# guangkun0818/speech2text

Hardware: AMD Instinct MI355X
Metric: audio-seconds/sec (train step, zipformer pruned-RNN-T) (higher is better)
Workload: dtype f32; 1 GPU; C3 zipformer pruned-RNN-T train step: chunk_size -1, 500 BPE, prune_range 5 (fbank+fwd+bwd+allreduce+ScaledAdam); accumulate_grad_batches=1, gemm_arith=bf16x2/3, per_gpu_batch=64, global_batch=64, labels_per_utt=50, parallelism=dp1

## Files before the change

### include/s2t_mi355.h

```cpp
#ifndef S2T_MI355_H_
#define S2T_MI355_H_

#ifdef __cplusplus
extern "C" {
#endif

int s2t_fbank_f32(const float* pcm, long pcm_stride, const long* num_samples, int batch,
                  const float* window400, const float* twiddle512, const int* mel_off,
                  const int* mel_k0, const float* mel_w, int nnz, int num_mel, float eps,
                  float scale_in, const float* cmvn_mean, const float* cmvn_istd, float* out,
                  int max_frames, long* out_frames, void* stream);

#define S2T_CTC_MAX_LABELS 1023
long s2t_ctc_workspace_floats(int B, int T, int Umax);
int s2t_ctc_loss_fwd_bwd(const float* logits, const long* targets, long tgt_stride,
                         const long* in_len, const long* tgt_len, int B, int T, int V, int Umax,
                         int blank, int zero_infinity, const float* grad_scale, float* workspace,
                         float* loss_per_utt, float* grad_logits, void* stream);

int s2t_fill_f32(float* p, long n, float v, void* stream);
int s2t_rnnt_row_exp(const float* x, long rows, int C, float* probs, float* rowmax, void* stream);
int s2t_rnnt_simple_pxpy(const float* am, const float* lm, const float* am_max,
                         const float* lm_max, const float* nrm, const long* symbols,
                         const long* boundary, int B, int S, int T, int C, int blank, float* px,
                         float* py, void* stream);
int s2t_rnnt_simple_w(const float* dpx, const float* dpy, const float* nrm, const float* gscale,
                      int B, int S, int T, float* W, void* stream);
int s2t_rnnt_simple_bwd(const float* am_probs, const float* lm_probs, const float* G_am,
                        const float* G_lm, const float* dpx, const float* dpy,
                        const float* gscale, const long* symbols, int B, int S, int T, int C,
                        int blank, float* d_am, float* d_lm, int accumulate, void* stream);
int s2t_mutual_info_fwd(const float* px, const float* py, const long* boundary, int B, int S,
                        int T, float* p, float* ans, void* stream);
int s2t_mutual_info_bwd(const float* px, const float* py, const long* boundary, const float* p,
                        const float* ans_grad, int B, int S, int T, float* px_grad,
                        float* py_grad, void* stream);
int s2t_rnnt_prune_ranges(const float* px_grad, const float* py_grad, const long* boundary, int B,
                          int S, int T, int s_range, long* ranges, void* stream);
int s2t_rnnt_pruned_fwd(const float* am, const float* lm, const long* ranges,
                        const long* symbols, const long* boundary, int B, int S, int T, int C,
                        int R, int blank, int act, float* px, float* py, float* lse, void* stream);
int s2t_rnnt_pruned_bwd(const float* am, const float* lm, const long* ranges,
                        const long* symbols, const float* lse, const float* dpx, const float* dpy,
                        const float* gscale, int B, int S, int T, int C, int R, int blank, int act,
                        float* d_am, float* d_lm, int accumulate, void* stream);
int s2t_rnnt_lattice_fwd(const float* logits, const long* ranges, const long* symbols,
                         const long* boundary, int B, int S, int T, int V, int R, int blank,
                         float* px, float* py, float* lse, void* stream);
int s2t_rnnt_lattice_bwd(const float* logits, const long* ranges, const long* symbols,
                         const float* lse, const float* dpx, const float* dpy,
                         const float* gscale, int B, int S, int T, int V, int R, int blank,
                         float* d_logits, void* stream);


int s2t_swoosh_fwd(const float* x, float* y, long n, float offset, float constant, void* stream);
int s2t_swoosh_bwd(const float* x, const float* g, float* d, long n, float offset, void* stream);
int s2t_biasnorm_fwd(const float* x, const float* bias, const float* log_scale, long rows, int D,
                     float* y, float* scales, void* stream);
int s2t_biasnorm_fwd_tb(const float* x, const float* bias, const float* log_scale, int T, int B, int D,
                        float* y, float* scales, void* stream);
int s2t_biasnorm_bwd_tb(const float* x, const float* bias, const float* scales, const float* g, int T,
                        int B, int D, float* dx, float* dbias, float* dls, void* stream);
int s2t_norm_bypass_fwd(const float* x, const float* bias, const float* log_scale, const float* orig,
                        const float* bypass_scale, const float* fm, int B, long rows, int D, float* out,
                        float* scales, void* stream);
int s2t_norm_bypass_bwd(const float* x, const float* bias, const float* scales, const float* orig,
                        const float* bypass_scale, const float* g, const float* fm, int B, long rows, int D,
                        float* dx, float* d_orig, float* d_bypass_scale, float* dbias, float* dls,
                        void* stream);
int s2t_biasnorm_bwd(const float* x, const float* bias, const float* scales, const float* g,
                     long rows, int D, float* dx, float* dbias, float* dls, void* stream);
long s2t_balancer_bwd_workspace_floats(void);
int s2t_balancer_bwd(const float* x, long ldx, const float* g, long ldg, long rows, int C,
                     float min_mean, float max_mean, float min_rms, float max_rms,
                     float grad_scale, float* out, long ldo, float* workspace, int parity,
                     float act_off, void* stream);
int s2t_balancer_stats(const float* x, long ldx, long rows, int C, float* stats, void* stream);
int s2t_balancer_apply(const float* x, long ldx, const float* g, long ldg, long rows, int C,
                       float min_mean, float max_mean, float min_rms, float max_rms,
                       float grad_scale, float* out, long ldo, const float* stats, float act_off,
                       void* stream);


int s2t_zipconv_fwd(const float* u, long ld, int gate_off, const unsigned char* mask, int T, int B,
                    int C, int K, int chunk, const float* wc, const float* bc, const float* wk,
                    const float* bk, const float* scale, float* y, void* stream);
int s2t_zipconv_fwd_act(const float* u, long ld, int gate_off, const unsigned char* mask, int T, int B,
                        int C, int K, int chunk, const float* wc, const float* bc, const float* wk,
                        const float* bk, const float* scale, float* y, float* y_act, int act_kind,
                        void* stream);
int s2t_zipconv_bwd(const float* u, long ld, int gate_off, const unsigned char* mask, int T, int B,
                    int C, int K, int chunk, const float* wc, const float* wk, const float* bk,
                    const float* scale, const float* dy, float* du, float* dwc, float* dbc,
                    float* dwk, float* dbk, float* dscale, float* workspace, void* stream);
int s2t_zipconv_bwd_data(const float* u, long ld, int gate_off, const unsigned char* mask, int T,
                         int B, int C, int K, int chunk, const float* wc, const float* wk,
                         const float* bk, const float* scale, const float* dy, float* du,
                         void* stream);
int s2t_zipconv_bwd_params(const float* u, long ld, int gate_off, const unsigned char* mask, int T,
                           int B, int C, int K, int chunk, const float* wc, const float* wk,
                           const float* bk, const float* scale, const float* dy, float* dwc,
                           float* dbc, float* dwk, float* dbk, float* dscale, float* workspace,
                           void* stream);
long s2t_zipconv_bwd_workspace_floats(int T, int B, int C, int K);


int s2t_relpos_attn_fwd(const float* qkp, const float* pos, const unsigned char* kpm,
                        const unsigned char* amask, int T, int B, int H, int qd, int pd, float* W,
                        void* stream);
int s2t_relpos_attn_fwd_flag(const float* qkp, const float* pos, const unsigned char* kpm,
                             const unsigned char* amask, int T, int B, int H, int qd, int pd,
                             float* W, float pen_limit, float* pen_flag, void* stream);
int s2t_relpos_attn_bwd(const float* qkp, const float* pos, const unsigned char* kpm,
                        const unsigned char* amask, int T, int B, int H, int qd, int pd,
                        const float* W, const float* dW, const float* dW0, const float* dO1,
                        const float* V1, int dv1, const float* dO2, const float* V2, int dv2,
                        int delta_given, float* delta_ws, float* dqkp, float* dpos,
                        float* workspace, void* stream);
long s2t_relpos_attn_bwd_workspace_floats(int T, int B, int H, int pd);
int s2t_attn_apply(const float* W, const float* v, int T, int B, int H, int dv, int transpose,
                   float* out, void* stream);


long s2t_linear_wgrad_workspace_floats(int R, int N, int M);
int s2t_linear_wgrad(const float* g, long ldg, const float* a, long lda, int R, int N, int M,
                     float* dW, float* db, int accumulate, float* workspace, void* stream);

int s2t_whiten_metric(float* xtx, float* colsum, long n, int G, int cg, float* cov, float* mean,
                      float* scal, float* host_metric, float* workspace, void* stream);
int s2t_whiten_prep(const float* cov, const float* mean, const float* scal, int G, int cg, float* dcov,
                    float* bias, float* sums64, void* stream);
int s2t_gemm_x3p_sq(const float* A, long lda, const unsigned short* Bp, int N, int K, float* C, long ldc,
                    int M, const float* bias, const float* other, long ld_other, float* sums, int tile,
                    void* stream);
int s2t_sumsq64(const float* g, long numel, float* sums64, void* stream);
int s2t_whiten_combine64(const float* g, const float* pg, long numel, float grad_scale,
                         const float* sums64, float* out, void* stream);
int s2t_whiten_dcov(const float* cov, const float* mean, const float* scal, int G, int cg,
                    float* dcov, float* bias, float* sums, void* stream);
int s2t_whiten_apply(const float* g, const float* pg, long numel, float grad_scale, float* sums,
                     float* out, void* stream);
int s2t_limit_param_grad(const float* x, const float* g, float lo, float hi, long n, float* out,
                         void* stream);

int s2t_bestrq_labels(const float* feats, int B, int T, int F, const float* proj, int D,
                      const float* codebooks, int ncb, int K, int T2, long* labels, void* stream);


int s2t_col2im3x3_nhwc(const float* dc, int B, int H, int W, int C, int Ho, int Wo, int sh, int sw,
                       float* dx, void* stream);

int s2t_conv3x3_c1(int mode, const float* x, const float* w, const float* bias, const float* g, int B,
                   int H, int W, int pw, int CO, float* y, float* dw, float* db, float* dx,
                   void* stream);

int s2t_conv3x3_s2(int mode, const float* x, const float* w, const float* bias, const float* g, int B,
                   int H, int W, int CI, int CO, float* y, float* dx, void* stream);

int s2t_conv3x3_gemm(int mode, const float* x, int B, int H, int W, int C, int sh, int sw, int CO,
                     const float* w2_or_g, const float* bias, float* out, float* db, void* stream);

int s2t_dwconv2d_nhwc_fwd(const float* x, const float* wgt, const float* bias, int N, int H, int W,
                          int C, int KH, int KW, int flip, float* y, void* stream);
int s2t_dwconv2d_nhwc_fwd_add(const float* x, const float* wgt, const float* bias, const float* add,
                              int N, int H, int W, int C, int KH, int KW, int flip, float* y,
                              void* stream);
long s2t_dwconv2d_wgrad_workspace_floats(int N, int H, int C, int KH, int KW);
int s2t_dwconv2d_nhwc_wgrad(const float* x, const float* dy, int N, int H, int W, int C, int KH,
                            int KW, float* workspace, float* dw, float* db, void* stream);

int s2t_optim_chunk_elems(void);
int s2t_optim_segc_floats(void);
int s2t_seg_stats(const float* p, const float* g, const int* chunk_off, const int* chunk_len,
                  int nchunks, float* partial, void* stream);
int s2t_scaled_adam_coef(const float* partial, const int* seg_chunk_begin, const int* seg_len,
                         int nchunks_all, int seg_lo, int seg_hi, float lr, float beta1,
                         float beta2, float eps, float scalar_lr_scale, float param_min_rms,
                         float param_max_rms, float scalar_max, float clip_val,
                         float clipping_scale, int step, int size_update_period,
                         int clipping_update_period, float bc2, float bc2_size, float beta2c,
                         float* param_rms, float* scale_exp_avg_sq, float* scale_grads,
                         float* model_norms, float* fstate, int* istate, float* segstat,
                         float* segc, const float* skip, void* stream);
int s2t_scaled_adam_apply(float* p, float* g, float* delta, float* exp_avg_sq,
                          const int* chunk_off, const int* chunk_len, const int* chunk_seg,
                          int nchunks, const float* segc, int zero_grad, void* stream);

int s2t_gemm_f32(int mode, const float* A, long lda, const float* B, long ldb, float* C, long ldc,
                 int M, int N, int K, const float* bias, const float* resid, long ldr,
                 const float* act_src, long lds, int act_kind, int pro_a, int pro_b, float* colsum,
                 int accumulate, void* stream);

int s2t_gemm_f32_batched(int mode, const float* A, long lda, long sA, const float* B, long ldb, long sB,
                         float* C, long ldc, long sC, int M, int N, int K, int batch, void* stream);

int s2t_gemm_f32_sq(int mode, const float* A, long lda, const float* B, long ldb, float* C, long ldc,
                    int M, int N, int K, const float* bias, const float* other, long ld_other,
                    float* sums, void* stream);
int s2t_whiten_combine(const float* g, const float* pg, long numel, float grad_scale, const float* sums,
                       float* out, void* stream);

int s2t_gemm_f32_tiled(int mode, const float* A, long lda, const float* B, long ldb, float* C,
                       long ldc, int M, int N, int K, const float* bias, const float* resid,
                       long ldr, int tile, void* stream);

int s2t_tn_x3(int set);
int s2t_tn_w(int set);
int s2t_nn_x3(int set);

int s2t_gemm_xtx(const float* x, long ldx, int R, int C, int cg, float* xtx, long ldc,
                 float* colsum, void* stream);

typedef struct S2tTnProblem {
  const float* A;
  long lda;
  const float* B;
  long ldb;
  float* C;
  long ldc;
  int M, N, K;
  float* colsum;
  float alpha;
} S2tTnProblem;
int s2t_gemm_tn_grouped(int n, const S2tTnProblem* probs, void* stream);

int s2t_smoothed_nll_fwd(const float* logits, const long* labels, long rows, int K, float scale,
                         float t_other, float t_label, float c0, float* row_loss, float* lse,
                         void* stream);
int s2t_smoothed_nll_bwd(const float* logits, const long* labels, const float* lse,
                         const float* row_weight, long rows, int K, float scale, float t_other,
                         float t_label, float* grad, void* stream);

int s2t_ctc_greedy(const float* logits, const long* lengths, int B, int T, int V, int blank,
                   long* tokens, long* out_len, void* stream);
int s2t_rnnt_greedy_stateless(const float* am, const long* lengths, const float* emb,
                              const float* conv_w, const float* lin_w, const float* lin_b,
                              const float* pre_w, const float* pre_b, int B, int T, int V, int E,
                              int D, int ctx, int act, int max_token_step, int max_out, int blank,
                              long* tokens, long* out_len, void* stream);

long s2t_rnnt_beam_workspace_bytes(int B, int T, int V, int beam_size);
int s2t_rnnt_beam_stateless(const float* am, const long* lengths, const float* emb,
                            const float* conv_w, const float* lin_w, const float* lin_b,
                            const float* pre_w, const float* pre_b, int B, int T, int V, int E,
                            int D, int ctx, int act, int blank, int beam_size, int cutoff_top_k,
                            void* workspace, long* tokens, long* frames, long* out_len,
                            float* score, void* stream);

long s2t_rnnt_stream_state_bytes(int B, int V, int ctx, int beam_size, int max_tokens);
int s2t_rnnt_stream_reset(void* state, const int* rows, int B, int V, int ctx, int beam_size,
                          int max_tokens, int blank, void* stream);
int s2t_rnnt_greedy_stateless_chunk(const float* am, const long* chunk_len, const float* emb,
                                    const float* conv_w, const float* lin_w, const float* lin_b,
                                    const float* pre_w, const float* pre_b, int B, int Tc, int V,
                                    int E, int D, int ctx, int act, int max_token_step,
                                    int max_tokens, int blank, void* state, long* tokens,
                                    long* out_len, int* overflow, void* stream);
int s2t_rnnt_beam_stateless_chunk(const float* am, const long* chunk_len, const float* emb,
                                  const float* conv_w, const float* lin_w, const float* lin_b,
                                  const float* pre_w, const float* pre_b, int B, int Tc, int V, int E,
                                  int D, int ctx, int act, int blank, int beam_size,
                                  int cutoff_top_k, int max_tokens, void* state, long* tokens,
                                  long* frames, long* out_len, float* score, long* stable_len,
                                  int* overflow, void* stream);

#define S2T_RNNT_LSTM_MAX_HIDDEN 1024
#define S2T_RNNT_LSTM_MAX_LAYERS 8
#define S2T_RNNT_LSTM_MAX_VOCAB 8192
#define S2T_RNNT_LSTM_MAX_BEAM 16
typedef struct S2tLstmLayer {
  const float* x2g_w;
  const float* x2g_b;
  const float* p2g_w;
  const float *g_gamma, *g_beta;
  const float *c_gamma, *c_beta;
} S2tLstmLayer;
typedef struct S2tRnntLstmDesc {
  int V, E, H, D, inner, num_layers, layer_norm, act;
  float in_eps, lstm_eps, out_eps;
  int pad_;
  const float* emb;
  const float *in_gamma, *in_beta;
  S2tLstmLayer layers[S2T_RNNT_LSTM_MAX_LAYERS];
  const float *lin_w, *lin_b;
  const float *out_gamma, *out_beta;
  const float *pre_w, *pre_b;
  const float *out1_w, *out1_b;
  const float *out2_w, *out2_b;
} S2tRnntLstmDesc;
long s2t_rnnt_lstm_workspace_bytes(const S2tRnntLstmDesc* desc, int B, int T, int beam_size);
int s2t_lstm_pred_step(const S2tRnntLstmDesc* desc, int R, const int* tokens, const int* emit,
                       const int* parent, const float* h_in, const float* c_in, const float* lm_in,
                       float* h_out, float* c_out, float* lm_out, void* workspace, void* stream);
int s2t_rnnt_greedy_lstm(const S2tRnntLstmDesc* desc, const float* am, const long* lengths, int B,
                         int T, int max_token_step, void* workspace, long* tokens, long* out_len,
                         void* stream);
int s2t_rnnt_beam_lstm(const S2tRnntLstmDesc* desc, const float* am, const long* lengths, int B,
                       int T, int beam_size, int cutoff_top_k, void* workspace, long* tokens,
                       long* frames, long* out_len, float* score, void* stream);

int s2t_row_energy(const float* x, long stride, const long* len, int B, int D, int mode, float* out,
                   void* stream);
int s2t_mix(const float* src, long sstride, const long* slen, const float* noise, long nstride,
// ... 313 lines not shown
```

### speech2text_amd/zip_kernels.py

```python
import ctypes
import os

import torch
import torch.nn.functional as F

from . import _native as N
from . import flat
from . import planes

_SW = {True: (4.0, 0.035), False: (1.0, 0.313261687)}


def _dev(*ts):
    for t in ts:
        if t is not None and not t.is_cuda:
            raise RuntimeError("speech2text_amd zipformer kernels run on the GPU only "
                               "(no CPU fallback); got a CPU tensor")


def _c16(t):
    t = t.contiguous()
    if t.data_ptr() % 16:
        t = t.clone()
    return t
# ... 1525 lines not shown
        w2m = w2 if w2.dim() == 2 else w2.reshape(w2.shape[0], -1)
        g2 = _rows(g)
        grads2 = (None, None)
        if not wgrad_into(w2p, b2p, g2, a):
            dw, db = linear_wgrad(g2, a, b2p is not None)
            grads2 = (dw.view(w2.shape), db)
        if ctx.bal_cfg is not None:
            dh = lt_matmul(1, g2, w2m, act_src=h, act_kind="swoosh_l", bal=ctx.bal_cfg)
        else:
            dh = lt_matmul(1, g2, w2m, act_src=h, act_kind="swoosh_l")
        grads1 = (None, None)
        if not wgrad_into(w1p, b1p, dh, x2):
            dw, db = linear_wgrad(dh, x2, b1p is not None)
            grads1 = (dw.view(w1.shape), db)
        dx = lt_matmul(1, dh, w1m).view(ctx.xshape) if ctx.needs_input_grad[0] else None
        return dx, grads1[0], grads1[1], grads2[0], grads2[1], (g if ctx.has_res else None), None


def ffn_block(x, w1, b1, w2, b2, residual=None, balancer_cfg=None):
    if not x.is_cuda:
        raise RuntimeError("speech2text_amd.ffn_block needs device tensors (HIP path only)")
    return _FfnBlock.apply(x, w1, b1, w2, b2, residual, balancer_cfg)


class _LinearColPerm(torch.autograd.Function):

    @staticmethod
    def forward(ctx, x, weight, bias, f, c):
        wp = weight.detach().view(-1, c, f).permute(0, 2, 1).reshape(-1, f * c)
        x2 = _rows(x)
        y = lt_matmul(0, x2, wp, bias)
        ctx.save_for_backward(x2, wp)
        ctx.params = (weight, bias)
        ctx.cfg = (x.shape, f, c)
        return y.view(x.shape[:-1] + (wp.shape[0],))

    @staticmethod
    def backward(ctx, g):
        x2, wp = ctx.saved_tensors
        weight, bias = ctx.params
        xshape, f, c = ctx.cfg
        g2 = _rows(g)
        dx = lt_matmul(1, g2, wp).view(xshape) if ctx.needs_input_grad[0] else None

        def compute():
            dwp, db = linear_wgrad(g2, x2, bias is not None)
            return [dwp.view(-1, f, c).permute(0, 2, 1).reshape(weight.shape), db]
        dw, db = side_param_grads((weight, bias), compute, keep=(g2, x2))
        return dx, dw, db, None, None


def linear_col_perm(x, weight, bias, f, c):
    if not x.is_cuda:
        raise RuntimeError("speech2text_amd.linear_col_perm needs device tensors (HIP path only)")
    return _LinearColPerm.apply(x, weight, bias, f, c)


def linear_pass(x, weight, bias=None):
    return _LinearPass.apply(x, weight, bias)


def linear(x, weight, bias=None, residual=None):
    if not x.is_cuda:
        raise RuntimeError("speech2text_amd.linear needs device tensors (HIP path only)")
    return _Linear.apply(x, weight, bias, residual)


def _wgrad_splitk(a, g, chunk=16384):
    R = a.shape[0]
    S = R // chunk
    if S < 4:
        return a.t().mm(g)
    main = torch.bmm(a[:S * chunk].view(S, chunk, -1).transpose(1, 2),
                     g[:S * chunk].view(S, chunk, -1)).sum(dim=0)
    if S * chunk < R:
        main = main + a[S * chunk:].t().mm(g[S * chunk:])
    return main


def linear_big_m(x, weight, bias):
    return _Linear.apply(x, weight, bias, None)


def _conv3x3_wgrad_implicit(x, g, sh, sw, has_bias):
    B, H, W, C = x.shape
    Cout = g.shape[-1]
    dw2 = torch.zeros((Cout, 9 * C), dtype=torch.float32, device=x.device)
    db = torch.zeros((Cout,), dtype=torch.float32, device=x.device) if has_bias else None
    R = g.numel() // Cout
    N.PROF[0] and N.profile_note("s2t_conv3x3_gemm", 4.0 * (x.numel() + g.numel()), 2.0 * R * Cout * 9 * C)
    N.check(N.lib().s2t_conv3x3_gemm(2, N.fp(x), B, H, W, C, sh, sw, Cout, N.fp(g), None, N.fp(dw2),
                                     N.fp(db), N.stream()), "s2t_conv3x3_gemm(wgrad)")
    return dw2.view(Cout, 3, 3, C).permute(0, 3, 1, 2), db


def _implicit_ok(x, Cout, sh=1, sw=1):
    B, H, W, C = x.shape
    rows = B * ((H - 3) // sh + 1) * ((W - 3) // sw + 1)
    return x.is_cuda and C % 4 == 0 and Cout % 4 == 0 and x.numel() < (1 << 31) and rows >= 4


class _Conv3x3Nhwc(torch.autograd.Function):

    @staticmethod
    def forward(ctx, x, weight, bias, sh, sw):
        _dev(x, weight)
        x = x.contiguous().float()
        B, H, W, C = x.shape
        Cout = weight.shape[0]
        Ho, Wo = (H - 3) // sh + 1, (W - 3) // sw + 1
        w2 = weight.permute(0, 2, 3, 1).reshape(Cout, 9 * C)
        ctx.implicit = _implicit_ok(x, Cout, sh, sw)
        pp = None
        if ctx.implicit and C % 16 == 0 and Cout % 16 == 0:
            pp = planes.adhoc_pieces(w2.detach().contiguous(), 0)
        if pp is not None:
            y = torch.empty((B * Ho * Wo, Cout), dtype=torch.float32, device=x.device)
            amap = RowMap(Ho * Wo, Wo, H * W * C, sh * W * C, sw * C, 0)
            N.check(_x3p_map(x, amap, 3 * C, [0, W * C, 2 * W * C], pp, Cout, y, Cout, None, 0, B * Ho * Wo,
                             None if bias is None else bias.detach()), "s2t_gemm_x3p_map(fwd)")
            ctx.save_for_backward(x, weight)
        elif ctx.implicit:
            y = torch.empty((B * Ho * Wo, Cout), dtype=torch.float32, device=x.device)
            N.PROF[0] and N.profile_note("s2t_conv3x3_gemm", 4.0 * (x.numel() + y.numel()),
                           2.0 * y.numel() * 9 * C)
            N.check(N.lib().s2t_conv3x3_gemm(0, N.fp(x), B, H, W, C, sh, sw, Cout, N.fp(w2),
                                             N.fp(bias), N.fp(y), None, N.stream()),
                    "s2t_conv3x3_gemm")
            ctx.save_for_backward(x, weight)
        else:
            s = x.stride()
            cols = x.as_strided((B, Ho, Wo, 3, 3 * C), (s[0], s[1] * sh, s[2] * sw, s[1], 1)) \
                .reshape(B * Ho * Wo, 9 * C)
            y = lt_matmul(0, cols, w2, bias)
            ctx.save_for_backward(cols, weight)
        ctx.cfg = (B, H, W, C, Ho, Wo, sh, sw, bias is not None)
        ctx.params = (weight, bias)
        return y.view(B, Ho, Wo, Cout)

    @staticmethod
    def backward(ctx, dy):
        xc, weight = ctx.saved_tensors
        B, H, W, C, Ho, Wo, sh, sw, has_bias = ctx.cfg
        Cout = weight.shape[0]
        g = dy.reshape(B * Ho * Wo, Cout)
        g = g if g.is_contiguous() else g.contiguous()
        if ctx.implicit:
            dweight, db = side_param_grads(
                ctx.params, lambda: list(_conv3x3_wgrad_implicit(xc, g, sh, sw, has_bias)), keep=(xc, g))
        else:
            dwmat, db = linear_wgrad(g, xc, has_bias)
            dweight = dwmat.view(Cout, 3, 3, C).permute(0, 3, 1, 2)
        dx = None
        if ctx.needs_input_grad[0] and ctx.implicit and (sh, sw) == (1, 2) and Cout % 16 == 0 \
                and C >= 16 and g.numel() * 5 < (1 << 31):
            dx = _conv3x3_s12_dgrad_map(g.view(B, Ho, Wo, Cout), weight.detach(), H, W)
        elif ctx.needs_input_grad[0] and ctx.implicit and 9 * C * Cout >= (1 << 18):
            gy = g.view(B, Ho, Wo, Cout).permute(0, 3, 1, 2)
            xin = xc.permute(0, 3, 1, 2)
            wcl = weight.contiguous(memory_format=torch.channels_last)
            dxn = torch.ops.aten.convolution_backward(gy, xin, wcl, None, [sh, sw], [0, 0], [1, 1],
                                                      False, [0, 0], 1, [True, False, False])[0]
            dx = dxn.permute(0, 2, 3, 1)
        elif ctx.needs_input_grad[0]:
            w2 = weight.permute(0, 2, 3, 1).reshape(Cout, 9 * C)
            dc = lt_matmul(1, g, w2)
            dx = torch.empty((B, H, W, C), dtype=torch.float32, device=dy.device)
            N.PROF[0] and N.profile_note("s2t_col2im3x3_nhwc", 4.0 * (dc.numel() + dx.numel()))
            N.check(N.lib().s2t_col2im3x3_nhwc(N.fp(dc), B, H, W, C, Ho, Wo, sh, sw, N.fp(dx),
                                               N.stream()), "s2t_col2im3x3_nhwc")
        return dx, dweight, db, None, None


_CONV_MAP_DGRAD_TILE = 221


_PAD_BUF = {}


def _conv3x3_s12_dgrad_map(g, wd, H, W):
    B, Ho, Wo, Cout = g.shape
    C = wd.shape[1]
    key = (B, Ho, Wo, Cout, g.device.index)
    gp = _PAD_BUF.get(key)
    if gp is None:
        _PAD_BUF.clear()
        gp = _PAD_BUF[key] = torch.zeros((B, Ho + 4, Wo + 2, Cout), dtype=torch.float32, device=g.device)
    gp[:, 2:Ho + 2, 1:Wo + 1].copy_(g)
    Wp = Wo + 2
    dx = torch.empty((B, H, W, C), dtype=torch.float32, device=g.device)
    for pw in (0, 1):
        kws = (2, 0) if pw == 0 else (1,)
        bc = torch.cat([wd[:, :, kh, kw].t() for kh in (0, 1, 2) for kw in kws], dim=1).contiguous()
        pp = planes.adhoc_pieces(bc, 0)
        if pp is None:
            raise RuntimeError("conv3x3 (map, stride 1x2): class weight outside the piece kernel's rules")
        Wc = (W - pw + 1) // 2
        amap = RowMap(H * Wc, Wc, (Ho + 4) * Wp * Cout, Wp * Cout, Cout, (2 * Wp + 1) * Cout)
        segoff = [(-kh * Wp - (1 if pw == 0 else 0)) * Cout for kh in (0, 1, 2)]
        cmap = RowMap(H * Wc, Wc, H * W * C, W * C, 2 * C, pw * C)
        N.check(_x3p_map(gp, amap, len(kws) * Cout, segoff, pp, C, dx, C, cmap, dx.numel(), B * H * Wc, None,
                         tile=_CONV_MAP_DGRAD_TILE), "s2t_gemm_x3p_map(dgrad 1x2)")
    return dx


RowMap = N.struct("S2tRowMap")


_CONV_MAP_TILE = 22


def _x3p_map(a, amap, seg, segoff, pp, ncols, out, ldc, cmap, c_elems, M, bias, tile=None):
    tile = _CONV_MAP_TILE if tile is None else tile
    if tile >= 200 and (seg % 32 or N.lib().s2t_gemm_arith() != 2):
        tile -= 200
    so = (ctypes.c_long * len(segoff))(*segoff)
    N.PROF[0] and N.profile_note("s2t_gemm_x3p_map", 4.0 * (a.numel() + out.numel()) + 6.0 * ncols * seg * len(segoff),
                                 2.0 * M * ncols * seg * len(segoff))
    return N.lib().s2t_gemm_x3p_map(_vp(a), ctypes.byref(amap), seg, len(segoff), so, ctypes.c_void_p(pp), ncols,
                                    _vp(out), ldc, None if cmap is None else ctypes.byref(cmap), c_elems, M,
                                    _vp(bias), tile, N.stream())


class _Conv3x3S2Map(torch.autograd.Function):

    @staticmethod
    def forward(ctx, x, weight, bias):
        _dev(x, weight)
        x = x.contiguous().float()
        B, H, W, C = x.shape
        Cout = weight.shape[0]
        Ho, Wo = (H - 3) // 2 + 1, (W - 3) // 2 + 1
        w2 = weight.detach().permute(0, 2, 3, 1).reshape(Cout, 9 * C).contiguous()
        pp = planes.adhoc_pieces(w2, 0)
        if pp is None:
            raise RuntimeError("conv3x3 (map): weight shape outside the piece kernel's rules")
        M = B * Ho * Wo
        y = torch.empty((M, Cout), dtype=torch.float32, device=x.device)
        amap = RowMap(Ho * Wo, Wo, H * W * C, 2 * W * C, 2 * C, 0)
        N.check(_x3p_map(x, amap, 3 * C, [0, W * C, 2 * W * C], pp, Cout, y, Cout, None, 0, M,
                         None if bias is None else bias.detach()), "s2t_gemm_x3p_map(fwd)")
        ctx.save_for_backward(x, weight)
        ctx.params = (weight, bias)
        ctx.dims = (B, H, W, C, Ho, Wo, Cout)
        return y.view(B, Ho, Wo, Cout)

    @staticmethod
    def backward(ctx, dy):
        x, weight = ctx.saved_tensors
        B, H, W, C, Ho, Wo, Cout = ctx.dims
        g = dy.contiguous().float()
        has_bias = ctx.params[1] is not None
        dweight, db = side_param_grads(
            ctx.params, lambda: list(_conv3x3_wgrad_implicit(x, g.view(-1, Cout), 2, 2, has_bias)), keep=(x, g))
        dx = None
        if ctx.needs_input_grad[0]:
            gp = F.pad(g, (0, 0, 1, 1, 1, 1))
            dx = torch.empty((B, H, W, C), dtype=torch.float32, device=g.device)
            wd = weight.detach()
            P2 = Wo + 2
            for ph in (0, 1):
                for pw in (0, 1):
                    taps = [(kh, kw) for kh in ((0, 2) if ph == 0 else (1,)) for kw in ((0, 2) if pw == 0 else (1,))]
                    bc = torch.cat([wd[:, :, kh, kw].t() for kh, kw in taps], dim=1).contiguous()
                    pp = planes.adhoc_pieces(bc, 0)
                    if pp is None:
                        raise RuntimeError("conv3x3 (map): class weight outside the piece kernel's rules")
                    Hc, Wc = (H - ph + 1) // 2, (W - pw + 1) // 2
                    amap = RowMap(Hc * Wc, Wc, (Ho + 2) * P2 * Cout, P2 * Cout, Cout, (P2 + 1) * Cout)
                    segoff = [((-1 if kh == 2 else 0) * P2 + (-1 if kw == 2 else 0)) * Cout for kh, kw in taps]
                    cmap = RowMap(Hc * Wc, Wc, H * W * C, 2 * W * C, 2 * C, (ph * W + pw) * C)
                    N.check(_x3p_map(gp, amap, Cout, segoff, pp, C, dx, C, cmap, dx.numel(), B * Hc * Wc, None),
                            "s2t_gemm_x3p_map(dgrad)")
        return dx, dweight, db


def conv3x3_s2_map_ok(x, weight, stride):
    return (x.is_cuda and tuple(stride) == (2, 2) and x.shape[-1] % 16 == 0 and weight.shape[0] % 16 == 0
            and x.shape[1] >= 3 and x.shape[2] >= 3 and x.numel() < (1 << 29) and weight.shape[1] == x.shape[-1])


def conv3x3_s2_map(x, weight, bias):
    return _Conv3x3S2Map.apply(x, weight, bias)


class _Conv3x3C1(torch.autograd.Function):

    @staticmethod
    def forward(ctx, x, weight, bias, pw, grad_scale=None):
        _dev(x, weight)
        ctx.grad_scale = grad_scale
        x3 = x.reshape(x.shape[0], x.shape[1], x.shape[2]).contiguous().float()
        B, H, W = x3.shape
        CO = weight.shape[0]
        y = torch.empty((B, H - 2, W + 2 * pw - 2, CO), dtype=torch.float32, device=x.device)
        w = weight.contiguous().float()
        N.PROF[0] and N.profile_note("s2t_conv3x3_c1", 4.0 * (x3.numel() + y.numel()))
        N.check(N.lib().s2t_conv3x3_c1(0, N.fp(x3), N.fp(w), N.fp(bias), None, B, H, W, pw, CO,
                                       N.fp(y), None, None, None, N.stream()), "s2t_conv3x3_c1")
        ctx.save_for_backward(x3, w)
        ctx.cfg = (pw, bias is not None, x.shape)
        return y

    @staticmethod
    def backward(ctx, g):
        x3, w = ctx.saved_tensors
        pw, has_bias, xshape = ctx.cfg
        B, H, W = x3.shape
        CO = w.shape[0]
        g = g.contiguous().float()
        acc = torch.zeros(CO * 10, dtype=torch.float32, device=g.device)
        L = N.lib()
        N.PROF[0] and N.profile_note("s2t_conv3x3_c1", 4.0 * (x3.numel() + g.numel()))
        N.check(L.s2t_conv3x3_c1(1, N.fp(x3), None, None, N.fp(g), B, H, W, pw, CO, None, N.fp(acc),
                                 ctypes_off(acc, CO * 9), None, N.stream()), "s2t_conv3x3_c1(wgrad)")
        dx = None
        if ctx.needs_input_grad[0]:
            dx = torch.empty_like(x3)
            N.PROF[0] and N.profile_note("s2t_conv3x3_c1", 4.0 * (g.numel() + dx.numel()))
            N.check(L.s2t_conv3x3_c1(2, None, N.fp(w), None, N.fp(g), B, H, W, pw, CO, None, None,
                                     None, N.fp(dx), N.stream()), "s2t_conv3x3_c1(dgrad)")
            dx = dx.view(xshape)
        if ctx.grad_scale is not None:
            acc = acc * float(ctx.grad_scale)
# ... 153 lines not shown
```

Before: 18070 audio-seconds/sec.

## Add direct MFMA kernel for stride-(1,2) conv3x3 input gradient

Adds a dedicated HIP kernel for the input gradient of the stride-(1,2) 3x3 conv in the subsampling frontend. It stages a padded tile of dy in LDS, pre-splits the weights into bf16 hi/lo fragments, and applies only the taps that touch each output column parity using 3-pass bf16 MFMA. This replaces the padded-copy map path and avoids materialising intermediate buffers. It only runs when Cin is 32, Cout is at most 128, and the gemm arithmetic mode is bf16x3; otherwise it falls back to the old paths. Exchanges a precision mode fixed to bf16x3 for fewer memory passes.

```diff
diff --git a/include/s2t_mi355.h b/include/s2t_mi355.h
--- a/include/s2t_mi355.h
+++ b/include/s2t_mi355.h
@@ -149,6 +149,10 @@
 
 int s2t_col2im3x3_nhwc(const float* dc, int B, int H, int W, int C, int Ho, int Wo, int sh, int sw,
                        float* dx, void* stream);
+
+long s2t_conv3x3_s12_dgrad_work_bytes(int Cin, int Cout);
+int s2t_conv3x3_s12_dgrad(const float* dy, const float* weight, int B, int H, int W, int Cin, int Cout,
+                          float* dx, void* work, void* stream);
 
 int s2t_conv3x3_c1(int mode, const float* x, const float* w, const float* bias, const float* g, int B,
                    int H, int W, int pw, int CO, float* y, float* dw, float* db, float* dx,
diff --git a/speech2text_amd/csrc/conv_dgrad.hip b/speech2text_amd/csrc/conv_dgrad.hip
--- /dev/null
+++ b/speech2text_amd/csrc/conv_dgrad.hip
@@ -0,0 +1,243 @@
+#include "common.h"
+#include "conv_dgrad_index.h"
+#include "../../include/s2t_mi355.h"
+
+namespace {
+
+typedef float f32x16 __attribute__((ext_vector_type(16)));
+typedef float f32x2 __attribute__((ext_vector_type(2)));
+typedef float f32x4 __attribute__((ext_vector_type(4)));
+typedef unsigned u32x4 __attribute__((ext_vector_type(4)));
+typedef __bf16 bf16x2 __attribute__((ext_vector_type(2)));
+typedef __bf16 bf16x8 __attribute__((ext_vector_type(8)));
+typedef const __attribute__((address_space(1))) f32x4* gf32x4p;
+typedef const __attribute__((address_space(1))) u32x4* gu32x4p;
+
+__device__ __forceinline__ void split_pair2(float x0, float x1, unsigned& p0, unsigned& p1) {
+  f32x2 x = {x0, x1};
+  p0 = __builtin_bit_cast(unsigned, __builtin_convertvector(x, bf16x2));
+  f32x2 h = {__uint_as_float(p0 << 16), __uint_as_float(p0 & 0xFFFF0000u)};
+  x = x - h;
+  p1 = __builtin_bit_cast(unsigned, __builtin_convertvector(x, bf16x2));
+}
+__device__ __forceinline__ void split8_2(const f32x4 v0, const f32x4 v1, u32x4& hi, u32x4& lo) {
+  unsigned a0, a1, b0, b1, c0, c1, d0, d1;
+  split_pair2(v0.x, v0.y, a0, a1);
+  split_pair2(v0.z, v0.w, b0, b1);
+  split_pair2(v1.x, v1.y, c0, c1);
+  split_pair2(v1.z, v1.w, d0, d1);
+  hi = u32x4{a0, b0, c0, d0};
+  lo = u32x4{a1, b1, c1, d1};
+}
+
+__global__ void conv_dgrad_prep_kernel(const float* __restrict__ w, u32x4* __restrict__ img, int Cout) {
+  const int kcn = Cout / 16;
+  const int idx = blockIdx.x * blockDim.x + threadIdx.x;
+  if (idx >= 9 * kcn * 64) return;
+  const int lane = idx & 63, f = idx >> 6;
+  const int kc = f % kcn, tap = f / kcn;
+  const int kh = tap / 3, kw = tap - kh * 3;
+  const int r = lane & 31, hh = lane >> 5;
+  float v[8];
+#pragma unroll
+  for (int e = 0; e < 8; ++e) v[e] = w[cdg_w_off(kc * 16 + hh * 8 + e, r, kh, kw)];
+  u32x4 hi, lo;
+  split8_2(f32x4{v[0], v[1], v[2], v[3]}, f32x4{v[4], v[5], v[6], v[7]}, hi, lo);
+  img[cdg_wimg_frag(Cout, kh, kw, kc, 0) + lane] = hi;
+  img[cdg_wimg_frag(Cout, kh, kw, kc, 1) + lane] = lo;
+}
+
+#define CDG_TH 3
+#define CDG_KC_MAX 8
+#define CDG_STAGE_U 8
+
+template <int KCN>
+__device__ __forceinline__ void load_tap(gu32x4p img, int pw, int tap, int lane, u32x4 (&bf)[KCN][2]) {
+  int kh, kw;
+  cdg_tap(pw, tap, &kh, &kw);
+  gu32x4p p = img + cdg_wimg_frag(KCN * 16, kh, kw, 0, 0) + lane;
+#pragma unroll
+  for (int kc = 0; kc < KCN; ++kc) {
+    bf[kc][0] = p[kc * 128];
+    bf[kc][1] = p[kc * 128 + 64];
+  }
+}
+
+__device__ __forceinline__ f32x16 mfma3(const u32x4 ah, const u32x4 al, const u32x4 bh, const u32x4 bl, f32x16 acc) {
+  const bf16x8 a0 = __builtin_bit_cast(bf16x8, ah), a1 = __builtin_bit_cast(bf16x8, al);
+  const bf16x8 b0 = __builtin_bit_cast(bf16x8, bh), b1 = __builtin_bit_cast(bf16x8, bl);
+  acc = __builtin_amdgcn_mfma_f32_32x32x16_bf16(a1, b0, acc, 0, 0, 0);
+  acc = __builtin_amdgcn_mfma_f32_32x32x16_bf16(a0, b1, acc, 0, 0, 0);
+  acc = __builtin_amdgcn_mfma_f32_32x32x16_bf16(a0, b0, acc, 0, 0, 0);
+  return acc;
+}
+
+template <int KCN, bool TWO>
+__device__ __forceinline__ void tap_body(const unsigned char* p0, const unsigned char* p1, const u32x4 (&bf)[KCN][2],
+                                         f32x16& acc0, f32x16& acc1) {
+  constexpr int LO = KCN * 32;
+  u32x4 a[2][2], c[2][2];
+  a[0][0] = *(const u32x4*)p0;
+  a[0][1] = *(const u32x4*)(p0 + LO);
+  if (TWO) {
+    c[0][0] = *(const u32x4*)p1;
+    c[0][1] = *(const u32x4*)(p1 + LO);
+  }
+#pragma unroll
+  for (int kc = 0; kc < KCN; ++kc) {
+    const int cur = kc & 1, nxt = cur ^ 1;
+    if (kc + 1 < KCN) {
+      a[nxt][0] = *(const u32x4*)(p0 + (kc + 1) * 32);
+      a[nxt][1] = *(const u32x4*)(p0 + (kc + 1) * 32 + LO);
+      if (TWO) {
+        c[nxt][0] = *(const u32x4*)(p1 + (kc + 1) * 32);
+        c[nxt][1] = *(const u32x4*)(p1 + (kc + 1) * 32 + LO);
+      }
+    }
+    acc0 = mfma3(a[cur][0], a[cur][1], bf[kc][0], bf[kc][1], acc0);
+    if (TWO) acc1 = mfma3(c[cur][0], c[cur][1], bf[kc][0], bf[kc][1], acc1);
+  }
+}
+
+__device__ __forceinline__ void store_block(const CdgGeom& g, int b, int h0, int pw, int blk, int r, int hh,
+                                            const f32x16& acc, float* __restrict__ dx) {
+#pragma unroll
+  for (int q = 0; q < 16; ++q) {
+    const int row = (q & 3) + 8 * (q >> 2) + 4 * hh;
+    const long off = cdg_dx_off(g, b, h0, pw, blk * 32 + row);
+    if (off >= 0) dx[off + r] = acc[q];
+  }
+}
+
+template <int KCN>
+__global__ __launch_bounds__(CDG_THREADS, 2) void conv_dgrad_kernel(const float* __restrict__ dy_,
+                                                                     const u32x4* __restrict__ img_,
+                                                                     float* __restrict__ dx, const CdgGeom g) {
+  extern __shared__ __attribute__((aligned(16))) unsigned char patch[];
+  __builtin_amdgcn_s_setprio(3);
+  const int tid = threadIdx.x, lane = tid & 63, wave = tid >> 6;
+  const int r = lane & 31, hh = lane >> 5;
+  const int b = blockIdx.x / g.tiles, h0 = (blockIdx.x - b * g.tiles) * g.TH;
+  constexpr int Cout = KCN * 16;
+  gu32x4p img = (gu32x4p)img_;
+  const __attribute__((address_space(1))) float* dy = (const __attribute__((address_space(1))) float*)dy_;
+
+  const int rows = cdg_rows(g, h0);
+  const int nb0 = (rows * cdg_class_cols(g, 0) + 31) / 32, nb1 = (rows * cdg_class_cols(g, 1) + 31) / 32;
+  const int w0 = wave, w1 = CDG_WAVES - 1 - wave;
+  const int ng0 = nb0 > w0 ? (nb0 - w0 + 7) / 8 : 0, ng1 = nb1 > w1 ? (nb1 - w1 + 7) / 8 : 0;
+  const int ng = ng0 + ng1;
+
+  u32x4 bf[KCN][2], bn[KCN][2];
+  if (ng > 0) load_tap<KCN>(img, ng0 > 0 ? 0 : 1, 0, lane, bf);
+
+  const int items = cdg_stage_items(g, h0);
+  for (int base = 0; base < items; base += CDG_THREADS * CDG_STAGE_U) {
+    f32x4 v[CDG_STAGE_U][2];
+    int lo_[CDG_STAGE_U];
+#pragma unroll
+    for (int u = 0; u < CDG_STAGE_U; ++u) {
+      const int idx = base + u * CDG_THREADS + tid;
+      lo_[u] = -1;
+      v[u][0] = f32x4{0.f, 0.f, 0.f, 0.f};
+      v[u][1] = v[u][0];
+      if (idx < items) {
+        const long src = cdg_stage_src(g, b, h0, idx, &lo_[u]);
+        if (src >= 0) {
+          gf32x4p p = (gf32x4p)(dy + src);
+          v[u][0] = p[0];
+          v[u][1] = p[1];
+        }
+      }
+    }
+#pragma unroll
+    for (int u = 0; u < CDG_STAGE_U; ++u)
+      if (lo_[u] >= 0) {
+        u32x4 hi, lo;
+        split8_2(v[u][0], v[u][1], hi, lo);
+        *(u32x4*)(patch + lo_[u]) = hi;
+        *(u32x4*)(patch + lo_[u] + 2 * Cout) = lo;
+      }
+  }
+  __syncthreads();
+
+  for (int gi = 0; gi < ng; ++gi) {
+    const int pw = gi >= ng0 ? 1 : 0;
+    const int blk = pw ? w1 + 8 * (gi - ng0) : w0 + 8 * gi;
+    const bool two = blk + 4 < (pw ? nb1 : nb0);
+    const int a0 = cdg_a_base(g, h0, pw, blk, r, hh);
+    const int a1 = two ? cdg_a_base(g, h0, pw, blk + 4, r, hh) : a0;
+    const int ntap = cdg_ntaps(pw);
+    f32x16 acc0, acc1;
+#pragma unroll
+    for (int q = 0; q < 16; ++q) acc0[q] = acc1[q] = 0.f;
+    for (int tap = 0; tap < ntap; ++tap) {
+      const bool more = tap + 1 < ntap;
+      if (more) load_tap<KCN>(img, pw, tap + 1, lane, bn);
+      else if (gi + 1 < ng) load_tap<KCN>(img, gi + 1 >= ng0 ? 1 : 0, 0, lane, bn);
+      int kh, kw;
+      cdg_tap(pw, tap, &kh, &kw);
+      const int sh = cdg_tap_shift(g, kh, kw == 2 ? 1 : 0);
+      if (two) tap_body<KCN, true>(patch + a0 + sh, patch + a1 + sh, bf, acc0, acc1);
+      else tap_body<KCN, false>(patch + a0 + sh, patch + a1 + sh, bf, acc0, acc1);
+#pragma unroll
+      for (int kc = 0; kc < KCN; ++kc) {
+        bf[kc][0] = bn[kc][0];
+        bf[kc][1] = bn[kc][1];
+      }
+    }
+    store_block(g, b, h0, pw, blk, r, hh, acc0, dx);
+    if (two) store_block(g, b, h0, pw, blk + 4, r, hh, acc1, dx);
+  }
+}
+
+template <int KCN>
+int launch(const float* dy, const u32x4* img, float* dx, const CdgGeom& g, long lds, hipStream_t st) {
+  static bool attr = false;
+  if (!attr) {
+    hipError_t er = hipFuncSetAttribute(reinterpret_cast<const void*>(conv_dgrad_kernel<KCN>),
+                                        hipFuncAttributeMaxDynamicSharedMemorySize, 160 * 1024);
+    if (er != hipSuccess) return (int)er;
+    attr = true;
+  }
+  hipLaunchKernelGGL(conv_dgrad_kernel<KCN>, dim3(g.B * g.tiles), dim3(CDG_THREADS), (size_t)lds, st, dy, img, dx, g);
+  S2T_CHECK_LAUNCH();
+  return 0;
+}
+
+}
+
+extern "C" long s2t_conv3x3_s12_dgrad_work_bytes(int Cin, int Cout) {
+  if (Cin != CDG_CIN || Cout < 16 || Cout > 16 * CDG_KC_MAX || Cout % 16) return 0;
+  return cdg_wimg_bytes(Cout);
+}
+
+extern "C" int s2t_conv3x3_s12_dgrad(const float* dy, const float* weight, int B, int H, int W, int Cin, int Cout,
+                                     float* dx, void* work, void* stream) {
+  if (B <= 0) return 0;
+  if (Cin != CDG_CIN || Cout < 16 || Cout > 16 * CDG_KC_MAX || Cout % 16 || H < 3 || W < 3 || !work) return -2;
+  if (s2t_gemm_arith_of(1) != 2) return -2;
+  const long Ho = H - 2, Wo = (W - 3) / 2 + 1;
+  if ((long)B * Ho * Wo * Cout >= (1L << 31) || (long)B * H * W * Cin >= (1L << 31)) return -2;
+  static const long kLdsMax = 150 * 1024;
+  int TH = CDG_TH;
+  while (TH > 1 && cdg_lds_bytes(TH, (int)Wo, Cout) > kLdsMax) --TH;
+  const long lds = cdg_lds_bytes(TH, (int)Wo, Cout);
+  if (lds > kLdsMax) return -2;
+  const CdgGeom g = cdg_geom(B, H, W, Cout, TH);
+  if ((long)B * g.tiles >= (1L << 31)) return -2;
+  hipStream_t st = (hipStream_t)stream;
+  const int nprep = 9 * (Cout / 16) * 64;
+  hipLaunchKernelGGL(conv_dgrad_prep_kernel, dim3((nprep + 255) / 256), dim3(256), 0, st, weight, (u32x4*)work, Cout);
+  S2T_CHECK_LAUNCH();
+  switch (Cout / 16) {
+    case 1: return launch<1>(dy, (const u32x4*)work, dx, g, lds, st);
+    case 2: return launch<2>(dy, (const u32x4*)work, dx, g, lds, st);
+    case 3: return launch<3>(dy, (const u32x4*)work, dx, g, lds, st);
+    case 4: return launch<4>(dy, (const u32x4*)work, dx, g, lds, st);
+    case 5: return launch<5>(dy, (const u32x4*)work, dx, g, lds, st);
+    case 6: return launch<6>(dy, (const u32x4*)work, dx, g, lds, st);
+    case 7: return launch<7>(dy, (const u32x4*)work, dx, g, lds, st);
+    default: return launch<8>(dy, (const u32x4*)work, dx, g, lds, st);
+  }
+}
diff --git a/speech2text_amd/csrc/conv_dgrad_index.h b/speech2text_amd/csrc/conv_dgrad_index.h
--- /dev/null
+++ b/speech2text_amd/csrc/conv_dgrad_index.h
@@ -0,0 +1,77 @@
+#pragma once
+
+#if defined(__HIPCC__)
+#define CDG_HD __host__ __device__ __forceinline__
+#else
+#define CDG_HD inline
+#endif
+
+#define CDG_CIN 32
+#define CDG_THREADS 256
+#define CDG_WAVES 4
+
+struct CdgGeom {
+  int B, H, W, Cout;
+  int Ho, Wo;
+  int TH;
+  int tiles;
+  int PW;
+  int pix;
+};
+
+CDG_HD int cdg_pix_bytes(int Cout) { return 4 * Cout + 16; }
+CDG_HD long cdg_lds_bytes(int TH, int Wo, int Cout) { return (long)(TH + 2) * (Wo + 2) * cdg_pix_bytes(Cout); }
+
+CDG_HD CdgGeom cdg_geom(int B, int H, int W, int Cout, int TH) {
+  CdgGeom g;
+  g.B = B; g.H = H; g.W = W; g.Cout = Cout;
+  g.Ho = H - 2;
+  g.Wo = (W - 3) / 2 + 1;
+  g.TH = TH;
+  g.tiles = (H + TH - 1) / TH;
+  g.PW = g.Wo + 2;
+  g.pix = cdg_pix_bytes(Cout);
+  return g;
+}
+
+CDG_HD int cdg_rows(const CdgGeom& g, int h0) { return g.H - h0 < g.TH ? g.H - h0 : g.TH; }
+CDG_HD int cdg_class_cols(const CdgGeom& g, int pw) { return (g.W - pw + 1) / 2; }
+
+CDG_HD int cdg_stage_items(const CdgGeom& g, int h0) { return (cdg_rows(g, h0) + 2) * g.PW * (g.Cout / 8); }
+CDG_HD long cdg_stage_src(const CdgGeom& g, int b, int h0, int idx, int* lds_off) {
+  const int g8n = g.Cout / 8;
+  const int q = idx % g8n, p = idx / g8n;
+  const int c = p % g.PW, t = p / g.PW;
+  *lds_off = p * g.pix + q * 16;
+  const int hd = h0 - 2 + t, wd = c - 1;
+  if (hd < 0 || hd >= g.Ho || wd < 0 || wd >= g.Wo) return -1;
+  return (((long)b * g.Ho + hd) * g.Wo + wd) * g.Cout + q * 8;
+}
+
+CDG_HD int cdg_a_base(const CdgGeom& g, int h0, int pw, int blk, int r, int hh) {
+  const int wc = cdg_class_cols(g, pw);
+  int m = blk * 32 + r;
+  if (m >= cdg_rows(g, h0) * wc) m = 0;
+  const int i = m / wc, j = m - i * wc;
+  return ((i + 2) * g.PW + j + 1) * g.pix + hh * 16;
+}
+CDG_HD int cdg_tap_shift(const CdgGeom& g, int kh, int dj) { return -(kh * g.PW + dj) * g.pix; }
+
+CDG_HD int cdg_ntaps(int pw) { return pw == 0 ? 6 : 3; }
+CDG_HD void cdg_tap(int pw, int tap, int* kh, int* kw) {
+  if (pw == 0) { *kh = tap >> 1; *kw = (tap & 1) * 2; }
+  else { *kh = tap; *kw = 1; }
+}
+
+CDG_HD long cdg_dx_off(const CdgGeom& g, int b, int h0, int pw, int m) {
+  const int wc = cdg_class_cols(g, pw);
+  if (m >= cdg_rows(g, h0) * wc) return -1;
+  const int i = m / wc, j = m - i * wc;
+  return (((long)b * g.H + h0 + i) * g.W + 2 * j + pw) * CDG_CIN;
+}
+
+CDG_HD long cdg_wimg_bytes(int Cout) { return 9L * (Cout / 16) * 2 * 64 * 16; }
+CDG_HD int cdg_wimg_frag(int Cout, int kh, int kw, int kc, int piece) {
+  return ((((kh * 3 + kw) * (Cout / 16) + kc) * 2) + piece) * 64;
+}
+CDG_HD int cdg_w_off(int co, int ci, int kh, int kw) { return ((co * CDG_CIN + ci) * 3 + kh) * 3 + kw; }
diff --git a/speech2text_amd/zip_kernels.py b/speech2text_amd/zip_kernels.py
--- a/speech2text_amd/zip_kernels.py
+++ b/speech2text_amd/zip_kernels.py
@@ -1701,17 +1701,19 @@
             dwmat, db = linear_wgrad(g, xc, has_bias)
             dweight = dwmat.view(Cout, 3, 3, C).permute(0, 3, 1, 2)
         dx = None
-        if ctx.needs_input_grad[0] and ctx.implicit and (sh, sw) == (1, 2) and Cout % 16 == 0 \
-                and C >= 16 and g.numel() * 5 < (1 << 31):
-            dx = _conv3x3_s12_dgrad_map(g.view(B, Ho, Wo, Cout), weight.detach(), H, W)
-        elif ctx.needs_input_grad[0] and ctx.implicit and 9 * C * Cout >= (1 << 18):
+        if ctx.needs_input_grad[0] and ctx.implicit and (sh, sw) == (1, 2):
+            with gemm_class(CLS_D):
+                dx = _conv3x3_s12_dgrad_direct(g, weight.detach(), B, H, W)
+                if dx is None and Cout % 16 == 0 and C >= 16 and g.numel() * 5 < (1 << 31):
+                    dx = _conv3x3_s12_dgrad_map(g.view(B, Ho, Wo, Cout), weight.detach(), H, W)
+        if dx is None and ctx.needs_input_grad[0] and ctx.implicit and 9 * C * Cout >= (1 << 18):
             gy = g.view(B, Ho, Wo, Cout).permute(0, 3, 1, 2)
             xin = xc.permute(0, 3, 1, 2)
             wcl = weight.contiguous(memory_format=torch.channels_last)
             dxn = torch.ops.aten.convolution_backward(gy, xin, wcl, None, [sh, sw], [0, 0], [1, 1],
                                                       False, [0, 0], 1, [True, False, False])[0]
             dx = dxn.permute(0, 2, 3, 1)
-        elif ctx.needs_input_grad[0]:
+        elif dx is None and ctx.needs_input_grad[0]:
             w2 = weight.permute(0, 2, 3, 1).reshape(Cout, 9 * C)
             dc = lt_matmul(1, g, w2)
             dx = torch.empty((B, H, W, C), dtype=torch.float32, device=dy.device)
@@ -1719,6 +1721,25 @@
             N.check(N.lib().s2t_col2im3x3_nhwc(N.fp(dc), B, H, W, C, Ho, Wo, sh, sw, N.fp(dx),
                                                N.stream()), "s2t_col2im3x3_nhwc")
         return dx, dweight, db, None, None
+
+
+def _conv3x3_s12_dgrad_direct(g, wd, B, H, W):
+    Cout, C = wd.shape[0], wd.shape[1]
+    if os.environ.get("S2T_CONV_DGRAD_DIRECT", "1") == "0" or g.dtype is not torch.float32:
+        return None
+    nwork = int(N.lib().s2t_conv3x3_s12_dgrad_work_bytes(C, Cout))
+    if nwork <= 0 or N.lib().s2t_gemm_arith_of(CLS_D) != 2:
+        return None
+    wd = wd.contiguous().float()
+    work = torch.empty((nwork,), dtype=torch.uint8, device=g.device)
+    dx = torch.empty((B, H, W, C), dtype=torch.float32, device=g.device)
+    N.PROF[0] and N.profile_note("s2t_conv3x3_s12_dgrad", 4.0 * (g.numel() + dx.numel() + wd.numel()),
+                                 2.0 * B * H * C * Cout * (6 * ((W + 1) // 2) + 3 * (W // 2)))
+    rc = N.lib().s2t_conv3x3_s12_dgrad(N.fp(g), N.fp(wd), B, H, W, C, Cout, N.fp(dx), work.data_ptr(), N.stream())
+    if rc == -2:
+        return None
+    N.check(rc, "s2t_conv3x3_s12_dgrad")
+    return dx
 
 
 _CONV_MAP_DGRAD_TILE = 221
```

Result: faster. 18290 audio-seconds/sec, median of 5 (+1.2%).
